# linwe2012/CourseComputationalPhotography

Hardware: AMD Instinct MI355X
Metric: Gauss-Seidel pixel-updates/s on WxH 5-point Poisson grid (higher is better)
Workload: dtype f64

## Files before the change

coursecomputationalphotography_amd/csrc/ccp_grid.hip:

```cpp
#include "ccp_grid_kernels.hpp"
#include "ccp_grid_fused.hpp"
#include "ccp_grid_lex.hpp"
#include "ccp_cg.hpp"
#include "ccp_grid_cg.hpp"
#include "ccp_comm.hpp"

#include <algorithm>
#include <functional>
#include <cstring>
#include <chrono>
#include <vector>

using namespace ccp;

constexpr int kEdgeRing = 64;

struct ccp_grid {
    ccp_grid_desc desc{};
    Geom geom{};
    int ghost_top = 0, ghost_bottom = 0;
    bool shrink_top = false, shrink_bottom = false;
    int device = 0;
    hipStream_t stream = nullptr;
    hipStream_t stream2 = nullptr;
    hipEvent_t ev_main = nullptr, ev_side = nullptr;
    unsigned long long *edge_counter = nullptr;
    unsigned long long *edge_flag = nullptr;
    unsigned long long edge_epoch = 0;
    unsigned *edge_timeout = nullptr;
    unsigned long long edge_timeout_ticks = 200000000ull;
    int wait_mode = 0;
    bool edge_signal = true;
    ccp_comm *comm = nullptr;
    int up_rank = -1, down_rank = -1;
    int send_up = 0, send_down = 0;
    hipStream_t stream_comm = nullptr;
    hipEvent_t ev_comm = nullptr, ev_ready = nullptr;
    bool overlap = true;
    long exchanges = 0;
    DevBuf<double> x, b;
    DevBuf<double> cg_r, cg_p, cg_p2, cg_ap;
    DevBuf<CgState> cg_state;
    DevBuf<double> x_alt;
    bool allow_swap = false;
    bool masked = false;
    DevBuf<unsigned char> maskp, tile_live;
    DevBuf<int> tile_rows;
    int live_T = -1, live_R = -1, live_lo = -1, live_hi = -1;
    long unknowns = 0;
    bool fuse = true;
    int multi = 0;
    DevBuf<unsigned> multi_words;
    bool xcd_swizzle = false;
    const char *trace_file = nullptr;
    DevBuf<unsigned long long> trace;
    bool short_edges = true;
    int side_rows_override = 0;
    int fuse_tmax = kFusedMaxT;
    int rows_per_chunk = 128;
    float tune_ms[kFusedMaxT + 1] = {0};
    int tune_rows[kFusedMaxT + 1] = {0};
    bool tuned = false;
    bool all_border = false;
    bool force_border = false;
    bool red_store_all = false;
    DevBuf<double> partial;
    long partial_region = 0;
    DevBuf<double> small;
    DevBuf<double> sweep_sums;
    DevBuf<SolveState> state;
    DevBuf<int> redo_mask;
    DevBuf<double> lex_x, lex_b, lex_snap, lex_partial, lex_eps;
    DevBuf<unsigned> lex_progress, lex_ticket;
    DevBuf<double> lex_edges;
    int lex_mode = 3;
    int lex_tmax = 8;
    unsigned *lex_order_pin = nullptr;
    unsigned *lex_order_dev = nullptr;
    size_t lex_order_pin_cap = 0;
    size_t lex_order_count = 0;
    int lex_order_groups = 0, lex_order_strips = 0, lex_order_depth = 0;
    LexGeom lexg{};
    DevBuf<double> stage;
    long stage_rows = 0;
    int half_sweeps_since_refresh = 0;
    hipEvent_t ev0 = nullptr, ev1 = nullptr;
    hipEvent_t ev_r0 = nullptr, ev_r1 = nullptr;
    long region_launches = 0;
    long region_iterations = 0;
    float last_ms = 0.f;
    int last_launches = 0;
    bool timing_pending = false;
    int cpt = 2;
    int rows_per_block = 32;
};

namespace {

int edge_timeout_status(const ccp_grid *g)
{
    if (g->edge_timeout && __atomic_load_n(g->edge_timeout, __ATOMIC_ACQUIRE) != 0) {
        if (getenv("CCP_GS_DEBUG")) fprintf(stderr, "[ccp_gs] an edge hand-off timed out: ghost rows may hold rows that were not final\n");
        return CCP_ERR_STATE;
    }
    return CCP_OK;
}

int bind(ccp_grid *g)
{
    if (!g) return CCP_ERR_BAD_ARG;
    if (hipSetDevice(g->device) != hipSuccess) return CCP_ERR_NO_DEVICE;
    return edge_timeout_status(g);
}

long sweep_blocks_x(const ccp_grid *g) { return (g->geom.pitch + (long)kBlock * g->cpt - 1) / ((long)kBlock * g->cpt); }

void choose_tiling(ccp_grid *g)
{
    const long bx = sweep_blocks_x(g);
    long r = (long)g->geom.local_rows * bx * g->desc.channels / 4096;
    r = std::max<long>(4, std::min<long>(64, r));
    g->rows_per_block = (int)r;
}

template <bool L1>
int launch_half_sweep(ccp_grid *g, int c, int l_lo, int l_hi, const int *active)
{
    if (l_hi <= l_lo) return CCP_OK;
    const Geom &geo = g->geom;
    const int rpb = g->rows_per_block;
    dim3 grid((unsigned)sweep_blocks_x(g), (unsigned)((l_hi - l_lo + rpb - 1) / rpb), (unsigned)g->desc.channels);
    dim3 block(kBlock);
    double *part = g->partial.p + (long)c * g->partial_region;
#define CCP_LAUNCH_SWEEP(CPT_, SHFL_)                                                                          \
    hipLaunchKernelGGL((k_half_sweep<CPT_, L1, SHFL_>), grid, block, 0, g->stream, g->x.p, g->x.p, g->b.p, geo, \
                       c, l_lo, l_hi, rpb, part, active, static_cast<const unsigned char *>(nullptr))
    if (g->masked) {
        hipLaunchKernelGGL((k_half_sweep<2, L1, true, true>), grid, block, 0, g->stream, g->x.p, g->x.p, g->b.p, geo, c, l_lo, l_hi,
                           rpb, part, active, g->maskp.p);
    } else {
        CCP_LAUNCH_SWEEP(2, true);
    }
#undef CCP_LAUNCH_SWEEP
    CCP_HIP(hipGetLastError());
    g->last_launches++;
    g->region_launches++;
    return CCP_OK;
}

void sweep_range(const ccp_grid *g, int &l_lo, int &l_hi)
{
    const int s = g->half_sweeps_since_refresh;
    l_lo = g->shrink_top ? std::min(s + 1, g->ghost_top) : 0;
    l_hi = g->geom.local_rows - (g->shrink_bottom ? std::min(s + 1, g->ghost_bottom) : 0);
}

long l1_blocks_per_colour_channel(const ccp_grid *g, int l_lo, int l_hi)
{
    const int rpb = g->rows_per_block;
    return sweep_blocks_x(g) * (long)((l_hi - l_lo + rpb - 1) / rpb);
}

int one_iteration(ccp_grid *g, bool l1, const int *active, long *blocks_out)
{
    for (int c = 0; c < 2; ++c) {
        int lo, hi;
        sweep_range(g, lo, hi);
        if ((g->shrink_top || g->shrink_bottom) && g->half_sweeps_since_refresh >= g->desc.ghost)
            return CCP_ERR_STATE;
        if (l1) {
            CCP_TRY(launch_half_sweep<true>(g, c, lo, hi, active));
            if (blocks_out) blocks_out[c] = l1_blocks_per_colour_channel(g, lo, hi);
        } else {
            CCP_TRY(launch_half_sweep<false>(g, c, lo, hi, active));
        }
        if (g->shrink_top || g->shrink_bottom) g->half_sweeps_since_refresh++;
    }
    return CCP_OK;
}

void fused_tile_counts(const ccp_grid *g, int T, FusedParams &P, int edge_rows = 0)
{
    const Geom &geo = g->geom;
    const int HS = 2 * T, R = P.rows_per_chunk;
    const int rows = P.st_hi - P.st_lo;
    const int edge_short = HS + 16;
    const bool at_top = geo.y0 + P.st_lo - HS <= 0, at_bot = geo.y0 + P.st_hi + HS >= geo.H - 1;
    const bool short_edges = g->short_edges;
    P.first_rows = (short_edges && at_top && rows > 2 * edge_short + R / 2 && R > edge_short) ? edge_short : 0;
    P.last_rows = (short_edges && at_bot && rows > 2 * edge_short + R / 2 && R > edge_short) ? edge_short : 0;
    P.first_edge = P.last_edge = 0;
    if (edge_rows > 0) {
        int want_top = (g->shrink_top && !at_top) ? geo.own_lo + std::min(edge_rows, g->send_up > 0 ? g->send_up : edge_rows) - P.st_lo : 0;
        int want_bot = (g->shrink_bottom && !at_bot) ? P.st_hi - (geo.own_hi - std::min(edge_rows, g->send_down > 0 ? g->send_down : edge_rows)) : 0;
        want_top += want_top & 1;
        want_bot += want_bot & 1;
        const int others = P.first_rows + P.last_rows;
        if (want_top > 0 && want_bot > 0 && rows < want_top + want_bot + others + 2) want_top = want_bot = 0;
        if (want_top > 0 && rows >= want_top + others + 2 && P.first_rows == 0) {
            P.first_rows = want_top;
            P.first_edge = 1;
        }
        if (want_bot > 0 && rows >= want_bot + P.first_rows + 2 && P.last_rows == 0) {
            P.last_rows = want_bot;
            P.last_edge = 1;
        }
    }
    const int mid = rows - P.first_rows - P.last_rows;
    if (P.first_edge || P.last_edge) {
        const int n_whole = (rows + R - 1) / R;
        const int n_mid = std::max(1, n_whole - P.first_edge - P.last_edge);
        int r_mid = (mid + n_mid - 1) / n_mid;
        r_mid += r_mid & 1;
        P.rows_per_chunk = std::max(R, r_mid);
    }
    P.n_chunks = (mid + P.rows_per_chunk - 1) / P.rows_per_chunk + (P.first_rows > 0) + (P.last_rows > 0);
    auto top = [&](int c) { int ra, rb; fused_chunk_rows(P, c, ra, rb); return geo.y0 + ra - HS <= 0; };
    auto bot = [&](int c) { int ra, rb; fused_chunk_rows(P, c, ra, rb); return geo.y0 + rb + HS >= geo.H - 1; };
    P.nb_top = 0;
    while (P.nb_top < P.n_chunks && top(P.nb_top)) ++P.nb_top;
    P.nb_bot = 0;
    while (P.nb_top + P.nb_bot < P.n_chunks && bot(P.n_chunks - 1 - P.nb_bot)) ++P.nb_bot;
    const int U = fused_useful_px(T);
    auto left = [&](int s) { return s * U - fused_halo_px(T) <= 0; };
    auto right = [&](int s) { return s * U - fused_halo_px(T) + 2 * kStripLanes >= geo.W - 1; };
    P.ns_left = 0;
    while (P.ns_left < P.n_strips && left(P.ns_left)) ++P.ns_left;
    P.ns_right = 0;
    while (P.ns_left + P.ns_right < P.n_strips && right(P.n_strips - 1 - P.ns_right)) ++P.ns_right;
    if (g->all_border) {
        P.nb_top = P.n_chunks;
        P.nb_bot = 0;
    }
}

int masked_tile_census(ccp_grid *g, const FusedParams &P, int T)
{
    if (g->live_T != T || g->live_R != P.rows_per_chunk || g->live_lo != P.st_lo || g->live_hi != P.st_hi) {
        const size_t tiles = (size_t)P.n_chunks * P.n_strips;
        if (g->tile_live.n < tiles) CCP_TRY(g->tile_live.alloc(tiles));
        if (g->tile_rows.n < 2 * tiles) CCP_TRY(g->tile_rows.alloc(2 * tiles));
        hipLaunchKernelGGL(k_masked_tile_census, dim3((unsigned)P.n_strips, (unsigned)P.n_chunks), dim3(kWave), 0, g->stream, P, T,
                           g->tile_live.p, g->tile_rows.p);
        CCP_HIP(hipGetLastError());
        g->live_T = T;
        g->live_R = P.rows_per_chunk;
        g->live_lo = P.st_lo;
        g->live_hi = P.st_hi;
    }
    return CCP_OK;
}

template <int T>
int launch_fused_masked(ccp_grid *g, FusedParams &P, int l1, long *l1_blocks, bool store_red)
{
    if (T > kMaskedMaxT) return CCP_ERR_BAD_ARG;
    constexpr int TM = T <= kMaskedMaxT ? T : 1;
    const int rows = P.st_hi - P.st_lo;
    P.first_rows = P.last_rows = 0;
    P.first_edge = P.last_edge = 0;
    P.n_chunks = (rows + P.rows_per_chunk - 1) / P.rows_per_chunk;
    P.nb_top = P.nb_bot = P.ns_left = P.ns_right = 0;
    P.side_rows = P.rows_per_chunk;
    P.side_subs = 1;
    P.side_rows_edge = P.rows_per_chunk;
    P.edge_counter = nullptr;
    P.edge_flag = nullptr;
    P.edge_target = P.edge_epoch = 0;
    P.trace = nullptr;
    const int waves = kBlock / kWave;
    dim3 grid((unsigned)((P.n_strips + waves - 1) / waves), (unsigned)P.n_chunks, (unsigned)g->desc.channels);
    if (l1_blocks) {
        l1_blocks[0] = (long)grid.x * grid.y;
        l1_blocks[1] = 0;
    }
    CCP_TRY(masked_tile_census(g, P, T));
    static const bool clip_rows = !(getenv("CCP_GS_MASK_ROWS") && atoi(getenv("CCP_GS_MASK_ROWS")) == 0);
    const int *rows_p = clip_rows ? g->tile_rows.p : nullptr;
    if (l1 == 2 && T > kMaskedMaxCheckedT) return CCP_ERR_BAD_ARG;
    constexpr int TMC = T <= kMaskedMaxCheckedT ? T : 1;
    if (l1 == 2) hipLaunchKernelGGL((k_fused_sweep_masked<TMC, 2, kFusedUnroll>), grid, dim3(kBlock), 0, g->stream, P, g->tile_live.p, rows_p);
    else if (l1 == 1) hipLaunchKernelGGL((k_fused_sweep_masked<TM, 1, kFusedUnroll>), grid, dim3(kBlock), 0, g->stream, P, g->tile_live.p, rows_p);
    else if (!store_red) hipLaunchKernelGGL((k_fused_sweep_masked<TM, 0, kFusedUnroll, false>), grid, dim3(kBlock), 0, g->stream, P, g->tile_live.p, rows_p);
    else hipLaunchKernelGGL((k_fused_sweep_masked<TM, 0, kFusedUnroll>), grid, dim3(kBlock), 0, g->stream, P, g->tile_live.p, rows_p);
    CCP_HIP(hipGetLastError());
    g->last_launches++;
    g->region_launches++;
    g->region_iterations += T;
    return CCP_OK;
}

template <int T>
int launch_fused_t(ccp_grid *g, const double *xin, double *xout, int st_lo, int st_hi, const int *active,
                   int l1 = 0, long *l1_blocks = nullptr, int rows_override = 0, int edge_rows = 0, bool *signalled = nullptr,
                   bool store_red = true)
{
    FusedParams P;
    P.xin = xin;
    P.xout = xout;
    P.b = g->b.p;
    P.g = g->geom;
    P.st_lo = st_lo;
    P.st_hi = st_hi;
    P.rows_per_chunk = rows_override > 0 ? rows_override : ((g->tuned && g->tune_rows[T] > 0) ? g->tune_rows[T] : g->rows_per_chunk);
    const int U = fused_useful_px(T);
    P.n_strips = (g->geom.W + U - 1) / U;
    P.partial = g->partial.p;
    P.partial_border = g->partial.p + g->partial_region;
    P.active = active;
    P.xcd_swizzle = g->xcd_swizzle ? 1 : 0;
    const bool want_edge = edge_rows > 0 && l1 == 0 && active == nullptr && g->edge_counter && g->edge_signal;
    P.mask = g->maskp.p;
    if (l1 != 0 || edge_rows > 0) store_red = true;
    if (g->masked) return launch_fused_masked<T>(g, P, l1, l1_blocks, store_red);
    fused_tile_counts(g, T, P, want_edge ? edge_rows : 0);
    const int waves = kBlock / kWave;
    const int edge_chunks = std::min(P.nb_top + P.nb_bot, P.n_chunks);
    const int edge_strips = std::min(P.ns_left + P.ns_right, P.n_strips);
    {
        const int HS = 2 * T, R = P.rows_per_chunk;
        int sr = std::max(16, (R + 2 * HS) * 2 / 5 - 2 * HS);
        sr += sr & 1;
        if (g->side_rows_override > 0) sr = std::max(2, g->side_rows_override);
        P.side_rows = std::min(sr, R);
        P.side_subs = (R + P.side_rows - 1) / P.side_rows;
        P.side_rows_edge = std::min(P.side_rows, 16);
        if (P.first_edge || P.last_edge)
            P.side_subs = std::max(P.side_subs, (std::max(P.first_rows, P.last_rows) + P.side_rows_edge - 1) / P.side_rows_edge);
    }
    const long n_border = (long)edge_chunks * (P.n_strips - edge_strips) + (long)P.n_chunks * edge_strips * P.side_subs;
    const bool any_plain = edge_chunks < P.n_chunks && edge_strips < P.n_strips;
    dim3 grid((unsigned)((P.n_strips + waves - 1) / waves), (unsigned)P.n_chunks, (unsigned)g->desc.channels);
    dim3 bgrid((unsigned)((n_border + waves - 1) / waves), 1, (unsigned)g->desc.channels);
    if (l1_blocks) {
        l1_blocks[0] = any_plain ? (long)grid.x * grid.y : 0;
        l1_blocks[1] = n_border ? (long)bgrid.x : 0;
    }
    if (l1 == 2 && T > kFusedMaxCheckedT) return CCP_ERR_BAD_ARG;
    const bool edge = want_edge && (P.first_edge || P.last_edge);
    P.edge_counter = g->edge_counter;
    P.edge_flag = g->edge_flag;
    P.edge_epoch = g->edge_epoch;
    P.edge_target = 0;
    if (edge) {
        long waves_expected = 0;
        for (int c = 0; c < P.n_chunks; c += std::max(1, P.n_chunks - 1)) {
            if (!fused_is_edge_chunk(P, c)) continue;
            int ra, rb;
            fused_chunk_rows(P, c, ra, rb);
            const int subs = std::min(P.side_subs, (rb - ra + P.side_rows_edge - 1) / P.side_rows_edge);
            waves_expected += (P.n_strips - edge_strips) + (long)edge_strips * subs;
        }
        P.edge_target = (unsigned long long)waves_expected * g->desc.channels;
        if (g->edge_epoch % kEdgeRing == 0) CCP_HIP(hipMemsetAsync(g->edge_counter, 0, sizeof(unsigned long long) * kEdgeRing, g->stream));
        P.edge_counter = g->edge_counter + (g->edge_epoch % kEdgeRing);
    }
    if (signalled) *signalled = edge;
    const size_t trace_plain = (size_t)grid.x * grid.y * grid.z * waves * 4, trace_border = (size_t)bgrid.x * bgrid.z * waves * 4;
    unsigned long long *trace_p = nullptr, *trace_b = nullptr;
    if (g->trace_file) {
        if (g->trace.n < trace_plain + trace_border) CCP_TRY(g->trace.alloc(trace_plain + trace_border));
        CCP_HIP(hipMemsetAsync(g->trace.p, 0, (trace_plain + trace_border) * sizeof(unsigned long long), g->stream));
        trace_p = g->trace.p;
        trace_b = g->trace.p + trace_plain;
    }
    P.trace = trace_b;
    constexpr int TC = T <= kFusedMaxCheckedT ? T : 1;
    hipStream_t bstream = g->stream2;
    if (n_border) {
        CCP_HIP(hipEventRecord(g->ev_main, g->stream));
        CCP_HIP(hipStreamWaitEvent(bstream, g->ev_main, 0));
    }
    if (n_border && edge) {
        hipLaunchKernelGGL((k_fused_border<T, 0, kFusedUnroll, true>), bgrid, dim3(kBlock), 0, bstream, P, g->force_border ? 1 : 0);
    }
    if (any_plain) {
        P.trace = trace_p;
        if (l1 == 2) hipLaunchKernelGGL((k_fused_sweep<TC, 2, kFusedUnroll>), grid, dim3(kBlock), 0, g->stream, P);
        else if (l1 == 1) hipLaunchKernelGGL((k_fused_sweep<T, 1, kFusedUnroll>), grid, dim3(kBlock), 0, g->stream, P);
        else if (edge) hipLaunchKernelGGL((k_fused_sweep<T, 0, kFusedUnroll, true>), grid, dim3(kBlock), 0, g->stream, P);
        else if (!store_red) hipLaunchKernelGGL((k_fused_sweep<T, 0, kFusedUnroll, false, false>), grid, dim3(kBlock), 0, g->stream, P);
        else hipLaunchKernelGGL((k_fused_sweep<T, 0, kFusedUnroll>), grid, dim3(kBlock), 0, g->stream, P);
    }
    if (n_border) {
        const int fb = g->force_border ? 1 : 0;
        P.trace = trace_b;
        if (l1 == 2) hipLaunchKernelGGL((k_fused_border<TC, 2, kFusedUnroll>), bgrid, dim3(kBlock), 0, bstream, P, fb);
        else if (l1 == 1) hipLaunchKernelGGL((k_fused_border<T, 1, kFusedUnroll>), bgrid, dim3(kBlock), 0, bstream, P, fb);
        else if (!edge) hipLaunchKernelGGL((k_fused_border<T, 0, kFusedUnroll>), bgrid, dim3(kBlock), 0, bstream, P, fb);
        CCP_HIP(hipEventRecord(g->ev_side, bstream));
        CCP_HIP(hipStreamWaitEvent(g->stream, g->ev_side, 0));
    }
    CCP_HIP(hipGetLastError());
    if (g->trace_file) {
        CCP_HIP(hipStreamSynchronize(g->stream));
        std::vector<unsigned long long> host(trace_plain + trace_border);
        CCP_HIP(hipMemcpy(host.data(), g->trace.p, host.size() * sizeof(unsigned long long), hipMemcpyDeviceToHost));
        if (FILE *f = fopen(g->trace_file, "ab")) {
            const unsigned long long head[8] = {0x43435054524143ull, (unsigned long long)T, grid.x, grid.y, grid.z, bgrid.x, (unsigned long long)host.size(),
                                                (unsigned long long)P.rows_per_chunk};
            fwrite(head, sizeof(head), 1, f);
            fwrite(host.data(), sizeof(unsigned long long), host.size(), f);
            fclose(f);
        }
    }
    g->last_launches++;
    g->region_launches++;
    g->region_iterations += T;
    return CCP_OK;
}

template <int T>
int launch_fused_multi_t(ccp_grid *g, int n_passes, const double *xin, double *xout, const int *st_lo, const int *st_hi, int red_skip = 0)
{
    if (n_passes < 2 || n_passes > kMultiMaxPasses || g->trace_file) return CCP_ERR_UNSUPPORTED;
    if (g->masked && T > kMaskedMaxT) return CCP_ERR_UNSUPPORTED;
    FusedMultiParams M{};
    FusedParams &P = M.P;
    P.xin = xin;
    P.xout = xout;
    P.b = g->b.p;
    P.g = g->geom;
    P.st_lo = st_lo[0];
    P.st_hi = st_hi[0];
    P.rows_per_chunk = (g->tuned && g->tune_rows[T] > 0) ? g->tune_rows[T] : g->rows_per_chunk;
    const int U = fused_useful_px(T);
    P.n_strips = (g->geom.W + U - 1) / U;
    P.partial = g->partial.p;
    P.partial_border = g->partial.p + g->partial_region;
    P.active = nullptr;
    P.xcd_swizzle = 0;
    P.mask = g->maskp.p;
    P.trace = nullptr;
    const int HS = 2 * T;
    if (g->masked) {
        P.first_rows = P.last_rows = P.first_edge = P.last_edge = 0;
        P.n_chunks = (P.st_hi - P.st_lo + P.rows_per_chunk - 1) / P.rows_per_chunk;
        P.nb_top = P.nb_bot = P.ns_left = P.ns_right = 0;
        P.side_rows = P.side_rows_edge = P.rows_per_chunk;
        P.side_subs = 1;
        CCP_TRY(masked_tile_census(g, P, T));
    } else {
        fused_tile_counts(g, T, P, 0);
        const int R = P.rows_per_chunk;
        int sr = std::max(16, (R + 2 * HS) * 2 / 5 - 2 * HS);
        sr += sr & 1;
        if (g->side_rows_override > 0) sr = std::max(2, g->side_rows_override);
        P.side_rows = std::min(sr, R);
        P.side_subs = (R + P.side_rows - 1) / P.side_rows;
        P.side_rows_edge = P.side_rows;
    }
    P.edge_counter = nullptr;
    P.edge_flag = nullptr;
    P.edge_epoch = P.edge_target = 0;
    if (P.rows_per_chunk < HS || (P.first_rows > 0 && P.first_rows < HS) || (P.last_rows > 0 && P.last_rows < HS)) return CCP_ERR_UNSUPPORTED;
    for (int c = 0; c + 1 < P.n_chunks; ++c) {
        int ra, rb, rc, rd;
        fused_chunk_rows(P, c, ra, rb);
        fused_chunk_rows(P, c + 1, rc, rd);
        if (rb - ra < HS && rd - rc < HS) return CCP_ERR_UNSUPPORTED;
    }
    for (int q = 0; q < n_passes; ++q) {
        if (st_hi[q] <= st_lo[q] || st_lo[q] < st_lo[0] || st_hi[q] > st_hi[0]) return CCP_ERR_UNSUPPORTED;
        M.st_lo[q] = st_lo[q];
        M.st_hi[q] = st_hi[q];
    }
    const int waves = kBlock / kWave;
    const int edge_chunks = std::min(P.nb_top + P.nb_bot, P.n_chunks);
    const int edge_strips = std::min(P.ns_left + P.ns_right, P.n_strips);
    const long n_border = g->masked ? 0 : (long)edge_chunks * (P.n_strips - edge_strips) + (long)P.n_chunks * edge_strips * P.side_subs;
    M.n_passes = n_passes;
    M.red_skip = red_skip;
    M.gx = (P.n_strips + waves - 1) / waves;
    M.gy = P.n_chunks;
    M.bgx = (int)((n_border + waves - 1) / waves);
    M.channels = g->desc.channels;
    const size_t cells = (size_t)n_passes * M.channels * P.n_chunks * P.n_strips;
    if (g->multi_words.n < cells + 2) CCP_TRY(g->multi_words.alloc(cells + 2));
    CCP_HIP(hipMemsetAsync(g->multi_words.p, 0, (cells + 2) * sizeof(unsigned), g->stream));
    M.ticket = g->multi_words.p;
    M.cells = g->multi_words.p + 2;
    M.error = g->edge_timeout;
    M.tile_live = g->tile_live.p;
    const long total = (long)n_passes * (M.bgx + (long)M.gx * M.gy) * M.channels;
    if (total > 0x7fffffffL) return CCP_ERR_UNSUPPORTED;
    constexpr int TM = T <= kMaskedMaxT ? T : 1;
    if (g->masked) hipLaunchKernelGGL((k_fused_multi<TM, kFusedUnroll, true>), dim3((unsigned)total), dim3(kBlock), 0, g->stream, M);
    else hipLaunchKernelGGL((k_fused_multi<T, kFusedUnroll>), dim3((unsigned)total), dim3(kBlock), 0, g->stream, M);
    CCP_HIP(hipGetLastError());
    g->last_launches += n_passes;
    g->region_launches += n_passes;
    g->region_iterations += (long)T * n_passes;
    return CCP_OK;
}

template <int TMAX>
struct FusedMultiDepth {
    static int launch(int T, ccp_grid *g, int n, const double *xin, double *xout, const int *lo, const int *hi, int red_skip = 0)
    {
        if (T == TMAX) return launch_fused_multi_t<TMAX>(g, n, xin, xout, lo, hi, red_skip);
        return FusedMultiDepth<TMAX - 1>::launch(T, g, n, xin, xout, lo, hi, red_skip);
    }
};
template <>
struct FusedMultiDepth<0> {
    static int launch(int, ccp_grid *, int, const double *, double *, const int *, const int *, int = 0) { return CCP_ERR_UNSUPPORTED; }
};

template <int TMAX>
struct FusedDepth {
    static int launch(int T, ccp_grid *g, const double *xin, double *xout, int st_lo, int st_hi, const int *active,
                      int l1, long *l1_blocks, int rows_override = 0, int edge_rows = 0, bool *signalled = nullptr, bool store_red = true)
    {
        if (T == TMAX) return launch_fused_t<TMAX>(g, xin, xout, st_lo, st_hi, active, l1, l1_blocks, rows_override, edge_rows, signalled, store_red);
        return FusedDepth<TMAX - 1>::launch(T, g, xin, xout, st_lo, st_hi, active, l1, l1_blocks, rows_override, edge_rows, signalled, store_red);
    }
};
template <>
struct FusedDepth<0> {
    static int launch(int, ccp_grid *, const double *, double *, int, int, const int *, int, long *, int = 0, int = 0, bool * = nullptr, bool = true) { return CCP_ERR_BAD_ARG; }
};

__global__ void k_publish_flag(unsigned long long *flag, unsigned long long epoch)
{
    if (threadIdx.x == 0 && blockIdx.x == 0) __hip_atomic_store(flag, epoch, __ATOMIC_RELEASE, __HIP_MEMORY_SCOPE_SYSTEM);
}

__global__ void k_wait_flag(const unsigned long long *flag, unsigned long long epoch, unsigned long long ticks, unsigned *timed_out)
{
    if (threadIdx.x != 0 || blockIdx.x != 0) return;
    const unsigned long long t0 = wall_clock64();
    while (__hip_atomic_load(flag, __ATOMIC_ACQUIRE, __HIP_MEMORY_SCOPE_SYSTEM) < epoch) {
        __builtin_amdgcn_s_sleep(64);
        if (wall_clock64() - t0 > ticks) {
            __hip_atomic_store(timed_out, 1u, __ATOMIC_RELEASE, __HIP_MEMORY_SCOPE_SYSTEM);
            break;
        }
    }
}

void edge_epoch_begin(ccp_grid *g) { g->edge_epoch++; }

int edge_epoch_publish_after_pass(ccp_grid *g)
{
    if (!g->edge_flag) return CCP_OK;
    if (g->wait_mode == 0) {
        CCP_HIP(hipStreamWriteValue64(g->stream, g->edge_flag, g->edge_epoch, 0));
    } else {
        hipLaunchKernelGGL(k_publish_flag, dim3(1), dim3(64), 0, g->stream, g->edge_flag, g->edge_epoch);
        CCP_HIP(hipGetLastError());
    }
    return CCP_OK;
// ... 73 lines not shown
        p ^= 1;
    }
    std::sort(plan.begin(), plan.end(), std::greater<int>());
    auto stores_red = [&](size_t k) { return g->red_store_all || k + 1 >= plan.size() || (l1_last && k + 2 == plan.size()); };
    double *cur = g->x.p, *alt = g->x_alt.p;
    for (size_t k = 0; k < plan.size();) {
        if (g->multi && active == nullptr) {
            size_t j = k;
            while (j < plan.size() && plan[j] == plan[k] && (int)(j - k) < kMultiMaxPasses &&
                   !(j + 1 == plan.size() && (l1_last || edge_rows > 0)))
                ++j;
            const int n = (int)(j - k), T = plan[k];
            const bool shrinking = g->shrink_top || g->shrink_bottom;
            if (n >= 2 && !(shrinking && g->half_sweeps_since_refresh + 2 * T * n > g->desc.ghost)) {
                int lo[kMultiMaxPasses], hi[kMultiMaxPasses];
                for (int q = 0; q < n; ++q) {
                    const int s = g->half_sweeps_since_refresh + 2 * T * (q + 1);
                    lo[q] = g->shrink_top ? std::min(s, g->ghost_top) : 0;
                    hi[q] = g->geom.local_rows - (g->shrink_bottom ? std::min(s, g->ghost_bottom) : 0);
                }
                int red_skip = 0;
                while (red_skip < n && !stores_red(k + red_skip)) ++red_skip;
                const int st = FusedMultiDepth<kFusedMaxT>::launch(T, g, n, cur, alt, lo, hi, red_skip);
                if (st == CCP_OK) {
                    if (shrinking) g->half_sweeps_since_refresh += 2 * T * n;
                    if (n & 1) std::swap(cur, alt);
                    k = j;
                    continue;
                }
                if (st != CCP_ERR_UNSUPPORTED) return st;
            }
        }
        const bool last = k + 1 == plan.size();
        CCP_TRY(launch_fused(g, plan[k], cur, alt, active, (l1_last && last) ? 1 : 0, l1_blocks, last ? edge_rows : 0, stores_red(k)));
        std::swap(cur, alt);
        ++k;
    }
    if (cur != g->x.p) {
        if (!free_parity) return CCP_ERR_STATE;
        std::swap(g->x.p, g->x_alt.p);
        std::swap(g->x.n, g->x_alt.n);
    }
    if (edge_rows > 0) CCP_TRY(edge_epoch_publish_after_pass(g));
    return CCP_OK;
}

__global__ void __launch_bounds__(kBlock)
k_zero_unmasked(double *__restrict__ p, const unsigned char *__restrict__ mask, long per_channel)
{
    double *__restrict__ q = p + (long)blockIdx.z * per_channel;
    for (long i = (long)blockIdx.x * kBlock + threadIdx.x; i < per_channel; i += (long)gridDim.x * kBlock)
        if (mask[i] == 0) q[i] = 0.0;
}

int zero_unmasked(ccp_grid *g, double *plane)
{
    if (!g->masked) return CCP_OK;
    hipLaunchKernelGGL(k_zero_unmasked, dim3(2048, 1, (unsigned)g->desc.channels), dim3(kBlock), 0, g->stream, plane, g->maskp.p,
                       g->geom.ch_stride);
    CCP_HIP(hipGetLastError());
    return CCP_OK;
}

int begin_timing(ccp_grid *g)
{
    g->last_launches = 0;
    g->timing_pending = false;
    CCP_HIP(hipEventRecord(g->ev0, g->stream));
    return CCP_OK;
}

int end_timing(ccp_grid *g)
{
    CCP_HIP(hipEventRecord(g->ev1, g->stream));
    g->timing_pending = true;
    return CCP_OK;
}

template <bool TO_DEVICE>
int transfer_rows(ccp_grid *g, double *dev_base, int channel, double *rows, int first_row, int n_rows)
{
    CCP_TRY(bind(g));
    if (!rows || channel < 0 || channel >= g->desc.channels || n_rows < 0) return CCP_ERR_BAD_ARG;
    const int img_lo = g->geom.y0, img_hi = g->geom.y0 + g->geom.local_rows;
    if (first_row < img_lo || first_row + n_rows > img_hi) return CCP_ERR_BAD_ARG;
    const int W = g->desc.width;
    int done = 0;
    while (done < n_rows) {
        const int chunk = (int)std::min<long>(g->stage_rows, n_rows - done);
        const int l_first = first_row + done - g->geom.y0;
        dim3 grid((unsigned)((W + kBlock - 1) / kBlock), (unsigned)chunk);
        const size_t bytes = (size_t)chunk * W * sizeof(double);
        double *host = rows + (size_t)done * W;
        if (TO_DEVICE) {
            CCP_HIP(hipMemcpyAsync(g->stage.p, host, bytes, hipMemcpyHostToDevice, g->stream));
            hipLaunchKernelGGL((k_convert<true>), grid, dim3(kBlock), 0, g->stream, dev_base, g->stage.p,
                               g->geom, channel, l_first, W);
            CCP_HIP(hipGetLastError());
        } else {
            hipLaunchKernelGGL((k_convert<false>), grid, dim3(kBlock), 0, g->stream, dev_base, g->stage.p,
                               g->geom, channel, l_first, W);
            CCP_HIP(hipGetLastError());
            CCP_HIP(hipMemcpyAsync(host, g->stage.p, bytes, hipMemcpyDeviceToHost, g->stream));
        }
        CCP_HIP(hipStreamSynchronize(g->stream));
        done += chunk;
    }
    return edge_timeout_status(g);
}

}

extern "C" {

int ccp_grid_create(const ccp_grid_desc *d, ccp_grid **out)
try {
    if (!d || !out) return CCP_ERR_BAD_ARG;
    *out = nullptr;
    if (d->width < 1 || d->height < 1 || d->channels < 1 || d->channels > kMaxChannels) return CCP_ERR_BAD_ARG;
    if (d->row_begin < 0 || d->row_count < 1 || d->row_begin + d->row_count > d->height || d->ghost < 0)
        return CCP_ERR_BAD_ARG;
    if ((long)d->width * d->height > 0x7fffffffL) return CCP_ERR_BAD_ARG;
    CCP_TRY(select_device(d->device));
    ccp_grid *g = new (std::nothrow) ccp_grid();
    if (!g) return CCP_ERR_ALLOC;
    g->desc = *d;
    g->device = d->device;
    g->ghost_top = d->row_begin > 0 ? std::min(d->ghost, d->row_begin) : 0;
    g->ghost_bottom = (d->row_begin + d->row_count < d->height) ? std::min(d->ghost, d->height - d->row_begin - d->row_count) : 0;
    Geom &geo = g->geom;
    geo.W = d->width;
    geo.H = d->height;
    geo.y0 = d->row_begin - g->ghost_top;
    g->shrink_top = geo.y0 > 0;
    g->shrink_bottom = d->row_begin + d->row_count + g->ghost_bottom < d->height;
    geo.local_rows = g->ghost_top + d->row_count + g->ghost_bottom;
    geo.own_lo = g->ghost_top;
    geo.own_hi = g->ghost_top + d->row_count;
    geo.pitch = (((long)d->width + 1) / 2 + 15) / 16 * 16;
    geo.ch_stride = (long)geo.local_rows * 2 * geo.pitch;
    g->cpt = 2;
    if (const char *e = getenv("CCP_GS_FUSE")) g->fuse = atoi(e) != 0;
    if (const char *e = getenv("CCP_GS_SHORT_EDGES")) g->short_edges = atoi(e) != 0;
    if (const char *e = getenv("CCP_GS_XCD")) g->xcd_swizzle = atoi(e) != 0;
    if (const char *e = getenv("CCP_GS_MULTI")) g->multi = atoi(e);
    if (const char *e = getenv("CCP_GS_TRACE_FILE")) g->trace_file = e[0] ? e : nullptr;
    if (const char *e = getenv("CCP_GS_SIDE_ROWS")) g->side_rows_override = atoi(e);
    if (const char *e = getenv("CCP_GS_LEX_MODE"))
        g->lex_mode = strcmp(e, "planes") == 0 ? 0 : 3;
    if (const char *e = getenv("CCP_GS_TMAX")) g->fuse_tmax = std::max(1, std::min(kFusedMaxT, atoi(e)));
    if (const char *e = getenv("CCP_GS_ALL_BORDER")) g->all_border = atoi(e) != 0;
    if (const char *e = getenv("CCP_GS_FORCE_BORDER")) g->force_border = atoi(e) != 0;
    if (const char *e = getenv("CCP_GS_RED_STORE")) g->red_store_all = atoi(e) != 0;
    if (const char *e = getenv("CCP_GS_CHUNK")) g->rows_per_chunk = std::max(1, atoi(e));
    choose_tiling(g);
    g->masked = (d->flags & CCP_GRID_DIRICHLET_MASK) != 0;
    if (g->masked) {
        g->fuse_tmax = std::min(g->fuse_tmax, kMaskedMaxT);
        if (!getenv("CCP_GS_CHUNK")) g->rows_per_chunk = 160;
    }

    const size_t elems = (size_t)geo.ch_stride * d->channels;
    int st = g->x.alloc(elems);
    if (st == CCP_OK && g->masked) {
        st = g->maskp.alloc((size_t)geo.ch_stride);
        if (st == CCP_OK && hipMemset(g->maskp.p, 0, (size_t)geo.ch_stride) != hipSuccess) st = CCP_ERR_HIP;
    }
    if (st == CCP_OK) st = g->b.alloc(elems);
    const size_t part = (size_t)((geo.pitch + 2L * kBlock - 1) / (2L * kBlock)) * geo.local_rows * d->channels * 2 * 2 + 64;
    g->partial_region = (long)(part / 2);
    if (st == CCP_OK) st = g->partial.alloc(part);
    if (st == CCP_OK) st = g->small.alloc(4 * kMaxChannels);
    if (st == CCP_OK) st = g->state.alloc(1);
    g->stage_rows = std::max<long>(1, std::min<long>(geo.local_rows, (8L << 20) / d->width));
    if (st == CCP_OK) st = g->stage.alloc((size_t)g->stage_rows * d->width);
    if (st == CCP_OK && (hipEventCreate(&g->ev0) != hipSuccess || hipEventCreate(&g->ev1) != hipSuccess)) st = CCP_ERR_HIP;
    if (st == CCP_OK && (hipStreamCreateWithFlags(&g->stream2, hipStreamNonBlocking) != hipSuccess ||
                         hipEventCreateWithFlags(&g->ev_main, hipEventDisableTiming) != hipSuccess ||
                         hipEventCreateWithFlags(&g->ev_side, hipEventDisableTiming) != hipSuccess))
        st = CCP_ERR_HIP;
    if (st == CCP_OK && (g->ghost_top || g->ghost_bottom)) {
        int can_wait = 0;
        (void)hipDeviceGetAttribute(&can_wait, hipDeviceAttributeCanUseStreamWaitValue, g->device);
        g->wait_mode = can_wait ? 0 : 1;
        if (const char *e = getenv("CCP_GS_EDGE_WAIT")) g->wait_mode = (strcmp(e, "spin") == 0) ? 1 : (can_wait ? 0 : 1);
        if (const char *e = getenv("CCP_GS_EDGE_SIGNAL")) g->edge_signal = atoi(e) != 0;
        if (hipMalloc(reinterpret_cast<void **>(&g->edge_counter), sizeof(unsigned long long) * kEdgeRing) != hipSuccess ||
            hipExtMallocWithFlags(reinterpret_cast<void **>(&g->edge_flag), sizeof(unsigned long long), hipMallocSignalMemory) != hipSuccess ||
            hipMemset(g->edge_counter, 0, sizeof(unsigned long long) * kEdgeRing) != hipSuccess ||
            hipMemset(g->edge_flag, 0, sizeof(unsigned long long)) != hipSuccess)
            st = CCP_ERR_HIP;
        if (const char *e = getenv("CCP_GS_EDGE_TIMEOUT_TICKS")) g->edge_timeout_ticks = strtoull(e, nullptr, 10);
    }
    if (st == CCP_OK && hipHostMalloc(reinterpret_cast<void **>(&g->edge_timeout), sizeof(unsigned), hipHostMallocMapped) != hipSuccess) st = CCP_ERR_HIP;
    if (g->edge_timeout) *g->edge_timeout = 0;
    if (st == CCP_OK && (hipMemset(g->x.p, 0, elems * sizeof(double)) != hipSuccess ||
                         hipMemset(g->b.p, 0, elems * sizeof(double)) != hipSuccess))
        st = CCP_ERR_HIP;
    if (st != CCP_OK) {
        ccp_grid_destroy(g);
        return st;
    }
    *out = g;
    return CCP_OK;
} CCP_ABI_CATCH

int ccp_grid_destroy(ccp_grid *g)
try {
    if (!g) return CCP_OK;
    (void)hipSetDevice(g->device);
    if (g->ev0) (void)hipEventDestroy(g->ev0);
    if (g->ev1) (void)hipEventDestroy(g->ev1);
    if (g->ev_r0) (void)hipEventDestroy(g->ev_r0);
    if (g->ev_r1) (void)hipEventDestroy(g->ev_r1);
    if (g->ev_main) (void)hipEventDestroy(g->ev_main);
    if (g->ev_side) (void)hipEventDestroy(g->ev_side);
    if (g->stream2) {
        (void)hipStreamSynchronize(g->stream2);
        (void)hipStreamDestroy(g->stream2);
    }
    if (g->stream_comm) {
        (void)hipStreamSynchronize(g->stream_comm);
        (void)hipStreamDestroy(g->stream_comm);
    }
    if (g->ev_comm) (void)hipEventDestroy(g->ev_comm);
    if (g->ev_ready) (void)hipEventDestroy(g->ev_ready);
    if (g->edge_counter) (void)hipFree(g->edge_counter);
    if (g->edge_flag) (void)hipFree(g->edge_flag);
    if (g->edge_timeout) (void)hipHostFree(g->edge_timeout);
    if (g->lex_order_pin) (void)hipHostFree(g->lex_order_pin);
    delete g;
    return CCP_OK;
} CCP_ABI_CATCH

int ccp_grid_get_layout(ccp_grid *g, ccp_grid_layout *out)
try {
    if (!g || !out) return CCP_ERR_BAD_ARG;
    out->x_dev = g->x.p;
    out->b_dev = g->b.p;
    out->pitch = g->geom.pitch;
    out->local_rows = g->geom.local_rows;
    out->ghost_top = g->ghost_top;
    out->ghost_bottom = g->ghost_bottom;
    out->channels = g->desc.channels;
    return CCP_OK;
} CCP_ABI_CATCH

int ccp_grid_set_stream(ccp_grid *g, void *hip_stream)
try {
    if (!g) return CCP_ERR_BAD_ARG;
    g->stream = reinterpret_cast<hipStream_t>(hip_stream);
    return CCP_OK;
} CCP_ABI_CATCH

int ccp_grid_synchronize(ccp_grid *g)
try {
    CCP_TRY(bind(g));
    CCP_HIP(hipStreamSynchronize(g->stream));
    return edge_timeout_status(g);
} CCP_ABI_CATCH

int ccp_grid_set_b_host(ccp_grid *g, int32_t channel, const double *rows, int32_t first_row, int32_t n_rows)
try {
    if (!g) return CCP_ERR_BAD_ARG;
    CCP_TRY(transfer_rows<true>(g, g->b.p, channel, const_cast<double *>(rows), first_row, n_rows));
    return zero_unmasked(g, g->b.p);
} CCP_ABI_CATCH

int ccp_grid_set_x_host(ccp_grid *g, int32_t channel, const double *rows, int32_t first_row, int32_t n_rows)
try {
    if (!g) return CCP_ERR_BAD_ARG;
    CCP_TRY(transfer_rows<true>(g, g->x.p, channel, const_cast<double *>(rows), first_row, n_rows));
    return zero_unmasked(g, g->x.p);
} CCP_ABI_CATCH

int ccp_grid_get_x_host(ccp_grid *g, int32_t channel, double *rows, int32_t first_row, int32_t n_rows)
try {
    if (!g) return CCP_ERR_BAD_ARG;
    return transfer_rows<false>(g, g->x.p, channel, rows, first_row, n_rows);
} CCP_ABI_CATCH

int ccp_grid_get_b_host(ccp_grid *g, int32_t channel, double *rows, int32_t first_row, int32_t n_rows)
try {
    if (!g) return CCP_ERR_BAD_ARG;
    return transfer_rows<false>(g, g->b.p, channel, rows, first_row, n_rows);
} CCP_ABI_CATCH

int ccp_grid_set_mask_host(ccp_grid *g, const uint8_t *mask, int64_t row_stride_bytes)
try {
    CCP_TRY(bind(g));
    if (!g->masked) return CCP_ERR_STATE;
    if (!mask || row_stride_bytes < g->desc.width) return CCP_ERR_BAD_ARG;
    const Geom &geo = g->geom;
    std::vector<unsigned char> split((size_t)geo.ch_stride, 0);
    long count = 0;
    for (int l = 0; l < geo.local_rows; ++l) {
        const int y = geo.y0 + l;
        const uint8_t *row = mask + (size_t)y * (size_t)row_stride_bytes;
        for (int x = 0; x < geo.W; ++x) {
            if (!row[x]) continue;
            split[(size_t)(((long)l * 2 + ((x + y) & 1)) * geo.pitch + (x >> 1))] = 1;
            if (l >= geo.own_lo && l < geo.own_hi) ++count;
        }
    }
    CCP_HIP(hipMemcpyAsync(g->maskp.p, split.data(), split.size(), hipMemcpyHostToDevice, g->stream));
    CCP_HIP(hipStreamSynchronize(g->stream));
// ... 1446 lines not shown
```

Before: 1947 billion.

## Add wide-lane fused Gauss-Seidel sweep kernel with LDS ring for RHS

Adds a new fused temporal-blocking sweep kernel for depth T=8 in which each lane handles two red and two black values via 128-bit buffer loads and stores. The right-hand side is pre-scaled and staged in a per-wave LDS ring buffer instead of being held in registers. Rows are double-buffered across a statically unrolled trip schedule. The goal is fewer memory instructions and fewer registers per useful pixel on the interior plain tiles, so more tiles fit and bandwidth is used better. The cost is extra halo overlap per wave, more LDS use, and one more code path that is on by default for T=8.

```diff
diff --git a/coursecomputationalphotography_amd/csrc/ccp_grid.hip b/coursecomputationalphotography_amd/csrc/ccp_grid.hip
--- a/coursecomputationalphotography_amd/csrc/ccp_grid.hip
+++ b/coursecomputationalphotography_amd/csrc/ccp_grid.hip
@@ -1,5 +1,6 @@
 #include "ccp_grid_kernels.hpp"
 #include "ccp_grid_fused.hpp"
+#include "ccp_grid_fused_wide.hpp"
 #include "ccp_grid_lex.hpp"
 #include "ccp_cg.hpp"
 #include "ccp_grid_cg.hpp"
@@ -64,6 +65,7 @@
     bool all_border = false;
     bool force_border = false;
     bool red_store_all = false;
+    bool wide = true;
     DevBuf<double> partial;
     long partial_region = 0;
     DevBuf<double> small;
@@ -356,7 +358,12 @@
         P.edge_counter = g->edge_counter + (g->edge_epoch % kEdgeRing);
     }
     if (signalled) *signalled = edge;
-    const size_t trace_plain = (size_t)grid.x * grid.y * grid.z * waves * 4, trace_border = (size_t)bgrid.x * bgrid.z * waves * 4;
+    const bool wide = T == kWideT && g->wide && l1 == 0 && !edge && any_plain;
+    const int wx0 = P.ns_left * U, wx1 = (P.n_strips - P.ns_right) * U;
+    const int n_wide = wide ? (wx1 - wx0 + wide_useful_px(T) - 1) / wide_useful_px(T) : 0;
+    const dim3 wgrid((unsigned)((n_wide + kWideWaves - 1) / kWideWaves), (unsigned)(P.n_chunks - edge_chunks), (unsigned)g->desc.channels);
+    const dim3 pgrid = wide ? wgrid : grid;
+    const size_t trace_plain = (size_t)pgrid.x * pgrid.y * pgrid.z * waves * 4, trace_border = (size_t)bgrid.x * bgrid.z * waves * 4;
     unsigned long long *trace_p = nullptr, *trace_b = nullptr;
     if (g->trace_file) {
         if (g->trace.n < trace_plain + trace_border) CCP_TRY(g->trace.alloc(trace_plain + trace_border));
@@ -379,6 +386,8 @@
         if (l1 == 2) hipLaunchKernelGGL((k_fused_sweep<TC, 2, kFusedUnroll>), grid, dim3(kBlock), 0, g->stream, P);
         else if (l1 == 1) hipLaunchKernelGGL((k_fused_sweep<T, 1, kFusedUnroll>), grid, dim3(kBlock), 0, g->stream, P);
         else if (edge) hipLaunchKernelGGL((k_fused_sweep<T, 0, kFusedUnroll, true>), grid, dim3(kBlock), 0, g->stream, P);
+        else if (wide && !store_red) hipLaunchKernelGGL((k_fused_sweep_wide<kWideT, false>), wgrid, dim3(kBlock), 0, g->stream, P, wx0, wx1, n_wide);
+        else if (wide) hipLaunchKernelGGL((k_fused_sweep_wide<kWideT, true>), wgrid, dim3(kBlock), 0, g->stream, P, wx0, wx1, n_wide);
         else if (!store_red) hipLaunchKernelGGL((k_fused_sweep<T, 0, kFusedUnroll, false, false>), grid, dim3(kBlock), 0, g->stream, P);
         else hipLaunchKernelGGL((k_fused_sweep<T, 0, kFusedUnroll>), grid, dim3(kBlock), 0, g->stream, P);
     }
@@ -397,7 +406,7 @@
         std::vector<unsigned long long> host(trace_plain + trace_border);
         CCP_HIP(hipMemcpy(host.data(), g->trace.p, host.size() * sizeof(unsigned long long), hipMemcpyDeviceToHost));
         if (FILE *f = fopen(g->trace_file, "ab")) {
-            const unsigned long long head[8] = {0x43435054524143ull, (unsigned long long)T, grid.x, grid.y, grid.z, bgrid.x, (unsigned long long)host.size(),
+            const unsigned long long head[8] = {0x43435054524143ull, (unsigned long long)T, pgrid.x, pgrid.y, pgrid.z, bgrid.x, (unsigned long long)host.size(),
                                                 (unsigned long long)P.rows_per_chunk};
             fwrite(head, sizeof(head), 1, f);
             fwrite(host.data(), sizeof(unsigned long long), host.size(), f);
@@ -777,6 +786,7 @@
     if (const char *e = getenv("CCP_GS_ALL_BORDER")) g->all_border = atoi(e) != 0;
     if (const char *e = getenv("CCP_GS_FORCE_BORDER")) g->force_border = atoi(e) != 0;
     if (const char *e = getenv("CCP_GS_RED_STORE")) g->red_store_all = atoi(e) != 0;
+    if (const char *e = getenv("CCP_GS_WIDE")) g->wide = atoi(e) != 0;
     if (const char *e = getenv("CCP_GS_CHUNK")) g->rows_per_chunk = std::max(1, atoi(e));
     choose_tiling(g);
     g->masked = (d->flags & CCP_GRID_DIRICHLET_MASK) != 0;
diff --git a/coursecomputationalphotography_amd/csrc/ccp_grid_fused_wide.hpp b/coursecomputationalphotography_amd/csrc/ccp_grid_fused_wide.hpp
--- /dev/null
+++ b/coursecomputationalphotography_amd/csrc/ccp_grid_fused_wide.hpp
@@ -0,0 +1,196 @@
+#pragma once
+
+#include "ccp_grid_fused.hpp"
+
+namespace ccp {
+
+constexpr int kWideT = 8;
+constexpr int kWideRing = 20;
+constexpr int kWideWaves = kBlock / kWave;
+__host__ __device__ constexpr int wide_useful_px(int T) { return 4 * kStripLanes - 4 * T; }
+
+typedef unsigned int u32x4 __attribute__((ext_vector_type(4)));
+typedef double d2 __attribute__((ext_vector_type(2)));
+
+__device__ __forceinline__ d2 buf_load2(__amdgpu_buffer_rsrc_t rs, unsigned voff)
+{
+    return __builtin_bit_cast(d2, __builtin_amdgcn_raw_buffer_load_b128(rs, (int)voff, 0, 0));
+}
+__device__ __forceinline__ void buf_store2(d2 v, __amdgpu_buffer_rsrc_t rs, unsigned voff)
+{
+    __builtin_amdgcn_raw_buffer_store_b128(__builtin_bit_cast(u32x4, v), rs, (int)voff, 0, 0);
+}
+
+struct WideCtx {
+    const double *__restrict__ xin;
+    double *__restrict__ xout;
+    const double *__restrict__ bb;
+    unsigned ld_r, ld_k;
+    unsigned st_r, st_k;
+    int ra, rb;
+    int m0, m1;
+    d2 *ring;
+};
+
+__device__ __forceinline__ void wide_load_row(const WideCtx &cx, const Geom &g, int q, d2 (&dst)[4])
+{
+    const bool exists = q >= cx.m0 && q < cx.m1;
+    const __amdgpu_buffer_rsrc_t rx = row_rsrc(cx.xin, g, q, exists), rbb = row_rsrc(cx.bb, g, q, exists);
+    dst[0] = buf_load2(rx, cx.ld_r);
+    dst[1] = buf_load2(rx, cx.ld_k);
+    dst[2] = buf_load2(rbb, cx.ld_r);
+    dst[3] = buf_load2(rbb, cx.ld_k);
+}
+
+__host__ __device__ constexpr int wide_slot(int k) { return ((k % kWideRing) + kWideRing) % kWideRing; }
+
+template <int T, bool STORE_RED, int NT, int PH>
+__device__ __forceinline__ void wide_step(d2 (&wr)[NT], d2 (&wk)[NT], const WideCtx &cx, const Geom &g, int f, int i)
+{
+    using Win = FusedWindow<T, 2>;
+    constexpr int HS = Win::HS;
+#pragma unroll
+    for (int h = 1; h <= HS; ++h) {
+        const int sr = Win::slot(i, h), su = Win::slot(i, h + 1), sd = Win::slot(i, h - 1);
+        const int c = (h - 1) & 1;
+        const int p = ((i - h + 2 * HS + 2) + c) & 1;
+        const d2 up = c ? wr[su] : wk[su];
+        const d2 dn = c ? wr[sd] : wk[sd];
+        const d2 o = c ? wr[sr] : wk[sr];
+        double la, ra, lb, rb;
+        if (p == 0) {
+            la = lane_prev(o.y); ra = o.x; lb = o.x; rb = o.y;
+        } else {
+            la = o.x; ra = o.y; lb = o.y; rb = lane_next(o.x);
+        }
+        const d2 bq = cx.ring[wide_slot(PH + i - h) * 2 * kWave + c * kWave];
+        d2 nv;
+        nv.x = __builtin_fma(((up.x + la) + ra) + dn.x, 0.25, bq.x);
+        nv.y = __builtin_fma(((up.y + lb) + rb) + dn.y, 0.25, bq.y);
+        if (c) wk[sr] = nv; else wr[sr] = nv;
+    }
+    {
+        const int r = f - HS;
+        const int sr = Win::slot(i, HS);
+        const __amdgpu_buffer_rsrc_t ro = row_rsrc(cx.xout, g, r, r >= cx.ra && r < cx.rb);
+        if constexpr (STORE_RED) buf_store2(wr[sr], ro, cx.st_r);
+        buf_store2(wk[sr], ro, cx.st_k);
+    }
+    __builtin_amdgcn_sched_barrier(0);
+}
+
+template <int NT>
+__device__ __forceinline__ void wide_place(d2 (&wr)[NT], d2 (&wk)[NT], const WideCtx &cx, int s0, int slot, const d2 (&row)[4])
+{
+    wr[s0] = row[0];
+    wk[s0] = row[1];
+    cx.ring[slot * 2 * kWave] = row[2] * 0.25;
+    cx.ring[slot * 2 * kWave + kWave] = row[3] * 0.25;
+}
+
+template <int T, bool STORE_RED, int NT, int PH>
+__device__ __forceinline__ void wide_trip(d2 (&wr)[NT], d2 (&wk)[NT], const WideCtx &cx, const Geom &g, int fb,
+                                          d2 (&landing)[2][4], const d2 (&arrived)[2][4])
+{
+    constexpr int G = 2;
+    using Win = FusedWindow<T, G>;
+#pragma unroll
+    for (int i = 0; i < G; ++i) wide_load_row(cx, g, fb + 2 * G + i, landing[i]);
+    __builtin_amdgcn_sched_barrier(0);
+#pragma unroll
+    for (int i = 0; i < G; ++i) {
+        if (i == 0) wide_step<T, STORE_RED, NT, PH>(wr, wk, cx, g, fb, 0);
+        else wide_step<T, STORE_RED, NT, PH>(wr, wk, cx, g, fb + 1, 1);
+    }
+#pragma unroll
+    for (int s = 0; s + G < NT; ++s) {
+        wr[s] = wr[s + G];
+        wk[s] = wk[s + G];
+    }
+#pragma unroll
+    for (int i = 0; i < G; ++i) wide_place(wr, wk, cx, Win::slot(i, 0), wide_slot(PH + G + i), arrived[i]);
+}
+
+template <int T, bool STORE_RED, int NT, int PH>
+__device__ __forceinline__ void wide_turn(d2 (&wr)[NT], d2 (&wk)[NT], const WideCtx &cx, const Geom &g, int fb,
+                                          d2 (&la)[2][4], d2 (&lb)[2][4])
+{
+    if constexpr (PH < kWideRing) {
+        if constexpr ((PH / 2) % 2 == 0) wide_trip<T, STORE_RED, NT, PH>(wr, wk, cx, g, fb, la, lb);
+        else wide_trip<T, STORE_RED, NT, PH>(wr, wk, cx, g, fb, lb, la);
+        wide_turn<T, STORE_RED, NT, PH + 2>(wr, wk, cx, g, fb + 2, la, lb);
+    }
+}
+
+template <int T, bool STORE_RED>
+__device__ __forceinline__ void fused_wave_wide(const double *__restrict__ xin, double *__restrict__ xout,
+                                                const double *__restrict__ bb, const Geom &g, int wx0, int wx1, int sw,
+                                                int ra, int rb, d2 *ring)
+{
+    static_assert(T % 2 == 0, "the lane pairs line up with the stored columns only for an even depth");
+    constexpr int G = 2;
+    static_assert(kWideRing % (2 * G) == 0 && kWideRing >= 2 * T + 2 * G, "the ring holds the rows a trip reads and the rows it lands");
+    using Win = FusedWindow<T, G>;
+    constexpr int HS = Win::HS, NT = Win::NT;
+    const int lane = (int)(threadIdx.x & (kWave - 1));
+    WideCtx cx;
+    cx.xin = xin; cx.xout = xout; cx.bb = bb;
+    cx.ring = ring + lane;
+    const int x0 = wx0 + sw * wide_useful_px(T);
+    const int x1 = min(x0 + wide_useful_px(T), wx1);
+    const int ja = (x0 - fused_halo_px(T)) / 2 + 2 * lane;
+    const bool col_ok = ja >= 0 && ja < g.pitch;
+    const bool col_store = col_ok && 2 * ja >= x0 && 2 * ja + 3 < x1;
+    cx.ld_r = col_ok ? (unsigned)ja * 8u : kLaneOut;
+    cx.ld_k = col_ok ? (unsigned)(g.pitch + ja) * 8u : kLaneOut;
+    cx.st_r = (STORE_RED && col_store) ? cx.ld_r : kLaneOut;
+    cx.st_k = col_store ? cx.ld_k : kLaneOut;
+    cx.ra = ra; cx.rb = rb;
+    cx.m0 = max(ra - HS, 0);
+    cx.m1 = min(rb + HS, g.local_rows);
+    const int base = cx.m0 - ((g.y0 + cx.m0) & 1);
+    const int f_end = rb - 1 + HS;
+
+    d2 wr[NT], wk[NT];
+    d2 la[G][4], lb[G][4];
+#pragma unroll
+    for (int s = 0; s < NT; ++s) wr[s] = wk[s] = d2{0.0, 0.0};
+#pragma unroll
+    for (int s = 0; s < kWideRing; ++s) {
+        cx.ring[s * 2 * kWave] = d2{0.0, 0.0};
+        cx.ring[s * 2 * kWave + kWave] = d2{0.0, 0.0};
+    }
+#pragma unroll
+    for (int i = 0; i < G; ++i) wide_load_row(cx, g, base + i, la[i]);
+#pragma unroll
+    for (int i = 0; i < G; ++i) wide_load_row(cx, g, base + G + i, lb[i]);
+#pragma unroll
+    for (int i = 0; i < G; ++i) wide_place(wr, wk, cx, Win::slot(i, 0), i, la[i]);
+    for (int fb = base; fb <= f_end; fb += kWideRing) wide_turn<T, STORE_RED, NT, 0>(wr, wk, cx, g, fb, la, lb);
+}
+
+template <int T, bool STORE_RED>
+__global__ void __launch_bounds__(kBlock, 2)
+k_fused_sweep_wide(FusedParams P, int wx0, int wx1, int n_wide)
+{
+    __shared__ d2 ring[kWideWaves][kWideRing * 2 * kWave];
+    const int wave = __builtin_amdgcn_readfirstlane(threadIdx.x / kWave);
+    unsigned bx, by, bz;
+    fused_tile_coords(P, bx, by, bz);
+    const int sw = (int)bx * kWideWaves + wave;
+    const int ch = (int)bz;
+    const int chunk = P.nb_top + (int)by;
+    int ra, rb;
+    fused_chunk_rows(P, chunk, ra, rb);
+    const bool run = (P.active == nullptr) || (P.active[ch] != 0);
+    if (run && sw < n_wide && ra < rb) {
+        const Geom &g = P.g;
+        const long off = (long)ch * g.ch_stride;
+        unsigned long long t0 = 0;
+        fused_trace_begin(P, t0);
+        fused_wave_wide<T, STORE_RED>(P.xin + off, P.xout + off, P.b + off, g, wx0, wx1, sw, ra, rb, ring[wave]);
+        fused_trace_end(P, t0, (((long)blockIdx.z * gridDim.y + blockIdx.y) * gridDim.x + blockIdx.x) * kWideWaves + wave, chunk, sw, ch, 3);
+    }
+}
+
+}
```

New measurement: 2103 billion (median of 6 runs). 8.0% higher.
